# MeteoSwiss/topo-descriptors

Hardware: AMD Instinct MI355X
Metric: Mpixels/s (and % HBM roofline) per descriptor, 1/2/4/8 MI355X (higher is better)
Workload: dtype f32

## Files before the change

### topo_descriptors_amd/csrc/disc_ring_wide_impl.hpp

```cpp
#pragma once

namespace topo {

namespace {

constexpr int NCW = 6;

template <int SIZE>
struct WGeo {
    static constexpr DiscTable<SIZE> T = make_disc_table<SIZE>();
    static_assert(T.centre == 0 && T.off_min == -T.off_max, "odd disc sizes only");
    static constexpr int M = T.off_max;
    static constexpr int DL = (M + NCW - 1) / NCW;
    static constexpr int NVL = 64 - 2 * DL;
    static constexpr int TILE_W = NCW * NVL;
    static constexpr int X0 = NCW * DL;
    static constexpr int W = 64 * NCW;
    static constexpr int NR = T.num_runs;
    static_assert(NVL >= 16, "disc too wide for one wavefront");
    struct Sched {
        int first_step[SIZE];
        int order[SIZE];
        int centre_run;
    };
    static constexpr Sched make() {
        Sched t{};
        for (int r = 0; r < SIZE; ++r) t.first_step[r] = -1;
        for (int r = 0; r < SIZE; ++r) t.order[r] = 0;
        t.centre_run = -1;
        for (int D = 0; D <= DL; ++D)
            for (int s = 0; s < NCW; ++s)
                for (int q = 0; q < NCW; ++q) {
                    const int dr = NCW * D + s - q, dl = -NCW * D + s - q;
                    if (dr >= 0 && dr <= M) {
                        const int r = T.run_of[dr - T.off_min];
                        if (D > t.first_step[r]) t.first_step[r] = D;
                    }
                    if (dl < 0 && dl >= -M) {
                        const int r = T.run_of[dl - T.off_min];
                        if (D > t.first_step[r]) t.first_step[r] = D;
                    }
                }
        int n = 0;
        for (int D = DL; D >= 0; --D)
            for (int d = M; d >= 0; --d) {
                const int r = T.run_of[d - T.off_min];
                bool seen = false;
                for (int i = 0; i < n; ++i) seen = seen || t.order[i] == r;
                if (!seen && t.first_step[r] == D) t.order[n++] = r;
            }
        for (int r = 0; r < NR; ++r)
            if (T.run_lo[r] == 0 && T.run_hi[r] == 0) t.centre_run = r;
        return t;
    }
    static constexpr Sched S = make();
    static_assert(S.centre_run >= 0, "the disc's outermost column is the pixel's own row");
};

template <int SIZE>
struct WideCfg {
    using G = WGeo<SIZE>;
    static constexpr int SW = 3;
    static constexpr int CW = 8;
    static constexpr int NW = SW + CW;
    static constexpr int RPW = 2;
    static constexpr int B = CW * RPW;
    static constexpr int TH = 64;
    static constexpr int PPT = TH / B;
    static constexpr int R = SIZE + 2 * B;
    static constexpr int HALO = SIZE - 1;
    static constexpr int PAD = 1 + (B - (1 + HALO + B) % B) % B;
    static constexpr int PRO = PAD + HALO + B;
    static constexpr int NB_PRO = PRO / B;
    static constexpr size_t LDS = (size_t)R * G::W * sizeof(uint32_t) + 2 * SW * sizeof(int) + 16;
    static_assert(SW * 128 == G::W, "two staged columns per staging lane");
    static_assert(TH % B == 0 && PRO % B == 0, "whole batches");
    static_assert(LDS <= 160 * 1024, "ring does not fit LDS");
    static_assert(NB_PRO <= 15, "batch history: two fields of a flag word");
};

constexpr bool tpi_wide_ring_fits(int size) {
    return size >= 5 && size % 2 == 1 && (size_t)(size + 32) * 384 * 4 + 64 <= 160 * 1024 && 64 - 2 * ((size / 2 + 5) / 6) >= 16;
}

__device__ __forceinline__ int wide_dword_of_column(int c) {
    const int l = c / NCW, s = c - NCW * l;
    return s < 4 ? 4 * l + s : 256 + 2 * l + (s - 4);
}

#ifndef WIDE_LEAD
#define WIDE_LEAD 2
#endif
#ifndef WIDE_PRIO
#define WIDE_PRIO 1
#endif

typedef uint32_t u32x2w __attribute__((ext_vector_type(2)));

template <int SIZE, int R, int LEAD>
__device__ __forceinline__ void wide_disc_sum(const uint32_t* ring, int s0, int lane, uint32_t (&acc)[NCW], uint32_t (&ctr)[NCW], bool first) {
    using G = WGeo<SIZE>;
    constexpr int NR = G::NR;
    constexpr int DL = G::DL;
    constexpr int M = G::M;
    constexpr uint32_t PB = (uint32_t)G::W * 4;
    constexpr uint32_t RB = (uint32_t)R * PB;
    u32x4 top4[NR], bot4[NR];
    u32x2w top2[NR], bot2[NR];
    uint32_t cv[NR][NCW];
    uint32_t aR[NCW], aL[NCW];
    const char* col4 = reinterpret_cast<const char*>(ring + lane * 4);
    const char* col2 = reinterpret_cast<const char*>(ring + 256 + lane * 2);
    const uint32_t b0 = (uint32_t)s0 * PB;
    auto fetch = [&](int i) {
        const int r = G::S.order[i];
        const uint32_t dt = (uint32_t)(G::T.run_hi[r] + 1 + M) * PB, db = (uint32_t)(G::T.run_lo[r] + M) * PB;
        const uint32_t ot = min(b0 + dt, b0 + dt - RB), ob = min(b0 + db, b0 + db - RB);
        top4[r] = *reinterpret_cast<const u32x4*>(col4 + ot);
        top2[r] = *reinterpret_cast<const u32x2w*>(col2 + ot);
        bot4[r] = *reinterpret_cast<const u32x4*>(col4 + ob);
        bot2[r] = *reinterpret_cast<const u32x2w*>(col2 + ob);
    };
#pragma unroll
    for (int i = 0; i < LEAD && i < NR; ++i) fetch(i);
#if WIDE_PRIO
    if (first) CHAIN_SETPRIO(3);
    else CHAIN_SETPRIO(1);
#endif
#pragma unroll
    for (int D = DL; D >= 0; --D) {
#if WIDE_PRIO
        if (D == DL / 2) {
            if (first) CHAIN_SETPRIO(2);
            else CHAIN_SETPRIO(0);
        }
#endif
#pragma unroll
        for (int j = 0; j < NR; ++j) {
            if (G::S.first_step[G::S.order[j]] == D) {
                const int r = G::S.order[j];
                if (j + LEAD < NR) fetch(j + LEAD);
                RING_SB();
#pragma unroll
                for (int s = 0; s < 4; ++s) cv[r][s] = top4[r][s] - bot4[r][s];
#pragma unroll
                for (int s = 0; s < 2; ++s) cv[r][4 + s] = top2[r][s] - bot2[r][s];
                RING_SB();
            }
        }
#pragma unroll
        for (int t = 0; t < NCW; ++t) {
            uint32_t pr = 0, pl = 0;
            bool anyr = false, anyl = false;
#pragma unroll
            for (int s = 0; s < NCW; ++s) {
                const int dr = NCW * D + s - t;
                const int dl = -NCW * D + s - t;
                if (dr >= 0 && dr <= M) {
                    const uint32_t c = cv[G::T.run_of[dr - G::T.off_min]][s];
                    pr = anyr ? pr + c : c;
                    anyr = true;
                }
                if (dl < 0 && dl >= -M) {
                    const uint32_t c = cv[G::T.run_of[dl - G::T.off_min]][s];
                    pl = anyl ? pl + c : c;
                    anyl = true;
                }
            }
            if (D == DL) {
                aR[t] = pr;
                aL[t] = pl;
            } else {
                if (anyr) {
                    asm("" : "+v"(pr));
                    aR[t] = hop(aR[t]) + pr;
                } else {
                    aR[t] = hop(aR[t]);
                }
                if (anyl) {
                    asm("" : "+v"(pl));
                    aL[t] = hop_up(aL[t]) + pl;
                } else {
                    aL[t] = hop_up(aL[t]);
                }
            }
        }
        RING_SB();
    }
#pragma unroll
    for (int t = 0; t < NCW; ++t) {
        acc[t] = aR[t] + aL[t];
        ctr[t] = cv[G::S.centre_run][t];
    }
}


template <int SIZE>
__global__ __launch_bounds__(WideCfg<SIZE>::NW * 64) void tpi_ring_wide_kernel(WaveArgs p, int tiles_x, int tiles_y, PartRun deal) {
    using G = WGeo<SIZE>;
    using C = WideCfg<SIZE>;
    constexpr int B = C::B, R = C::R, PPT = C::PPT, SW = C::SW, NB_PRO = C::NB_PRO, DL = G::DL;
    constexpr unsigned kWindow = (1u << NB_PRO) - 1u;
    constexpr int kBad = 1, kFracOnly = 1 << 15;
    constexpr unsigned kHistMask = kWindow | kWindow * kFracOnly;
    extern __shared__ __attribute__((aligned(16))) uint32_t lds_u[];
    uint32_t* Q = lds_u;
    int* wflags = reinterpret_cast<int*>(Q + R * G::W);

    const int nb = (int)gridDim.x;
    const int vb = (nb & 7) ? (int)blockIdx.x : (int)(blockIdx.x & 7) * (nb >> 3) + (int)(blockIdx.x >> 3);
    const int lane = threadIdx.x & 63;
    const int wave = __builtin_amdgcn_readfirstlane((int)(threadIdx.x >> 6));
    const int ntiles = tiles_x * tiles_y;
    const int first = deal.first(vb);
    const int last = min(first + deal.count(vb), ntiles);
    const double inv_nm1 = 1.0 / ((double)G::T.taps - 1.0);
    const int rmin = max(0, p.in_row0), rmax = min(p.gny, p.in_row0 + p.in_rows);
    const bool stager = wave < SW;
    const int scol = 128 * wave + 2 * lane;
    const int sdw0 = wide_dword_of_column(scol), sdw1 = wide_dword_of_column(scol + 1);
    int seen_tiles = 0, seen_frac = 0;

#pragma unroll 1
    for (int pos = first; pos < last;) {
        const int tile0 = pos;
        const int ty0 = tile0 % tiles_y;
        const int run_tiles = min(last - tile0, tiles_y - ty0);
        const int strip = tile0 / tiles_y;
        const int nphase = run_tiles * PPT;
        const int ox0 = strip * G::TILE_W;
        const int oyS = (p.out_row0 / C::TH + ty0) * C::TH;
        const int gx0 = ox0 - G::X0;
        const int gy0 = oyS - G::M - C::PAD;
        const int gcol = gx0 + scol;
        const bool col_ok = stager && gcol >= 0 && gcol < p.nx;
        const float* src = p.in + (col_ok ? gcol : 0);
        auto load_batch = [&](int n0, float2 (&v)[B]) {
#pragma unroll
            for (int r = 0; r < B; ++r) {
                int gy = gy0 + n0 + r;
                gy = min(max(gy, rmin), rmax - 1);
                v[r] = *reinterpret_cast<const float2*>(src + (size_t)(gy - p.in_row0) * p.nx);
            }
        };
        uint32_t run0 = 0, run1 = 0;
        int wslot = 0;
        const uint32_t kLimBits = __float_as_uint(kAbsLim + 1.0f);
        auto stage_batch = [&](int n0, const float2 (&v)[B]) {
            uint32_t amax = 0;
            bool frac = false;
#pragma unroll
            for (int r = 0; r < B; ++r) {
                const int gy = gy0 + n0 + r;
                const bool ok = col_ok && gy >= rmin && gy < rmax;
                const float x0 = ok ? v[r].x : 0.0f, x1 = ok ? v[r].y : 0.0f;
                const int i0 = (int)x0, i1 = (int)x1;
                const uint32_t a0 = __float_as_uint(x0) & 0x7fffffffu, a1 = __float_as_uint(x1) & 0x7fffffffu;
                frac |= x0 != (float)i0 || x1 != (float)i1;
                amax = max(amax, max(a0, a1));
                run0 += (uint32_t)i0;
                run1 += (uint32_t)i1;
                int sl = wslot + r;
                sl = sl >= R ? sl - R : sl;
                Q[sl * G::W + sdw0] = run0;
                Q[sl * G::W + sdw1] = run1;
            }
            const bool wild = __builtin_amdgcn_ballot_w64(amax >= kLimBits) != 0;
            const bool any_frac = __builtin_amdgcn_ballot_w64(frac) != 0;
            const bool bad = wild || any_frac;
            const bool fr = !wild && any_frac;
            return (bad ? kBad : 0) | (fr ? kFracOnly : 0);
        };
        auto advance_wslot = [&]() {
            wslot += B;
            wslot = wslot >= R ? wslot - R : wslot;
        };
        unsigned hist = 0;
        auto fold = [&](int parity) {
            int all = 0;
#pragma unroll
            for (int w = 0; w < SW; ++w) all |= wflags[parity * SW + w];
            all = __builtin_amdgcn_readfirstlane(all);
            hist = ((hist << 1) | (unsigned)all) & kHistMask;
        };

        float2 va[B];
        __syncthreads();
        if (stager) {
            int bits = 0;
#pragma unroll 1
            for (int k = 0; k < NB_PRO; ++k) {
                load_batch(k * B, va);
                bits |= stage_batch(k * B, va) << (NB_PRO - 1 - k);
                advance_wslot();
            }
            if (lane == 0) wflags[wave] = bits;
            load_batch(C::PRO, va);
        } else {
            for (int k = 0; k < NB_PRO; ++k) advance_wslot();
        }
        __syncthreads();
        {
            int all = 0;
#pragma unroll
            for (int w = 0; w < SW; ++w) all |= wflags[w];
            hist = (unsigned)__builtin_amdgcn_readfirstlane(all) & kHistMask;
        }

        const int ocol = gx0 + lane * NCW;
        const bool lane_ok = lane >= DL && lane < DL + G::NVL && ocol < p.nx;
        bool tile_frac = false;
#pragma unroll 1
        for (int ph = 0; ph < nphase; ++ph) {
            const bool compute = (hist & kWindow) == 0;
            const int oyA = oyS + ph * B;
            tile_frac = tile_frac || (hist & (kWindow * kFracOnly)) != 0;
            if (!compute) {
                const int r0 = max(oyA, p.out_row0), r1 = min(oyA + B, p.out_row0 + p.out_rows) - 1;
                if (r0 <= r1 && threadIdx.x == 0) {
                    const int base = p.out_row0 / p.map_th;
                    const int mx0 = ox0 / p.map_tw, mx1 = (min(ox0 + G::TILE_W, p.nx) - 1) / p.map_tw;
                    for (int mx = mx0; mx <= mx1; ++mx)
                        for (int my = r0 / p.map_th; my <= r1 / p.map_th; ++my) p.defer[mx * p.map_tiles_y + (my - base)] = kNeedsFraction;
                }
            }
            if (ph % PPT == PPT - 1) {
                ++seen_tiles;
                seen_frac += tile_frac ? 1 : 0;
                tile_frac = false;
            }
            if (stager) {
                const int seen = stage_batch(C::PRO + ph * B, va);
                if (lane == 0) wflags[((ph + 1) & 1) * SW + wave] = seen;
                load_batch(C::PRO + (ph + 1) * B, va);
            } else if (compute) {
#pragma unroll 1
                for (int k = 0; k < C::RPW; ++k) {
                    const int j = (wave - SW) * C::RPW + k;
                    const int oy = oyA + j;
                    if (oy < p.out_row0 || oy >= p.out_row0 + p.out_rows) continue;
                    const int s0 = (C::PAD - 1 + ph * B + j) % R;
                    uint32_t acc[NCW], ctr[NCW];
                    wide_disc_sum<SIZE, R, WIDE_LEAD>(Q, s0, lane, acc, ctr, k == 0);
                    if (lane_ok) {
                        float* o = p.tpi + (size_t)(oy - p.out_row0) * p.nx + ocol;
                        float out_t[NCW];
#pragma unroll
                        for (int t = 0; t < NCW; ++t) {
                            const int xi = (int)ctr[t];
                            out_t[t] = (float)((double)xi - (double)((int)acc[t] - xi) * inv_nm1);
                        }
#pragma unroll
                        for (int P = 0; P < NCW / 2; ++P)
                            if (ocol + 2 * P < p.nx) *reinterpret_cast<float2*>(o + 2 * P) = make_float2(out_t[2 * P], out_t[2 * P + 1]);
                    }
                }
            }
            advance_wslot();
            __syncthreads();
            fold((ph + 1) & 1);
        }
        pos += run_tiles;
    }
    if (p.report != nullptr && vb == nb / 2 && threadIdx.x == 0) {
        __hip_atomic_store(p.report + 1, (uint32_t)seen_frac, __ATOMIC_RELAXED, __HIP_MEMORY_SCOPE_SYSTEM);
        __hip_atomic_store(p.report, (uint32_t)seen_tiles, __ATOMIC_RELAXED, __HIP_MEMORY_SCOPE_SYSTEM);
    }
}

template <int SIZE>
int launch_ring_wide(const Block& b, float* tpi_out, int map_th, int map_tw) {
    using G = WGeo<SIZE>;
    using C = WideCfg<SIZE>;
    Context& c = ctx();
    TOPO_REQUIRE(c.seams.n == 0, "the wide ring takes single-block calls only");
    WaveArgs a{b.in, tpi_out, nullptr, b.in_rows, b.in_row0, b.gny, b.nx, b.out_row0, b.out_rows,
               nullptr, nullptr, nullptr, 0, 0, 0};
    static int blocks_per_cu = 0;
    if (blocks_per_cu == 0) {
        TOPO_HIP(hipFuncSetAttribute((const void*)tpi_ring_wide_kernel<SIZE>, hipFuncAttributeMaxDynamicSharedMemorySize, (int)C::LDS));
        int nblk = 0;
        TOPO_HIP(hipOccupancyMaxActiveBlocksPerMultiprocessor(&nblk, (const void*)tpi_ring_wide_kernel<SIZE>, C::NW * 64, C::LDS));
        blocks_per_cu = nblk < 1 ? 1 : nblk;
    }
    a.report = dem_memo_report(b);
    WaveParts ps;
    int tiles_x = 0;
    long ntiles = 0;
    TOPO_TRY(make_parts(b, a, C::TH, G::TILE_W, true, false, &ps, &tiles_x, &ntiles, map_th, map_tw));
    TOPO_REQUIRE(ps.n == 1 && ps.a[0].map_th == map_th && ps.a[0].map_tw == map_tw, "wide ring: tile map of another geometry");
    const size_t map_bytes = (size_t)((b.nx + map_tw - 1) / map_tw) * ps.a[0].map_tiles_y;
    TOPO_HIP(hipMemsetAsync(ps.a[0].defer, kTileDone, map_bytes, c.compute));
    const long grid = march_grid(c, blocks_per_cu, ntiles);
    deal_parts(&ps, tiles_x, grid, blocks_per_cu);
    hipLaunchKernelGGL(tpi_ring_wide_kernel<SIZE>, dim3((unsigned)grid), dim3(C::NW * 64), C::LDS, c.compute, ps.a[0], tiles_x, ps.tiles_y[0], ps.run[0]);
    TOPO_HIP(hipGetLastError());
    return TOPO_AMD_OK;
}

}

}
```

Before: 287,100.

## Share LDS base addresses across disc reads with a mirrored ring guard band

Stores each pixel's six columns contiguously in the LDS ring instead of in a split 4+2 dword layout. Adds GR guard rows that mirror the first ring rows, so nearby row reads can use one shared base register plus a constant offset with no per-read wrap. It also fuses the final left/right chain hop into a single step, turns the first-row flag into a template parameter and fully unrolls the two-row loop. The cost is extra LDS for the guard rows and duplicate stores for those rows, which narrows which disc sizes fit. The LDS reads change from 16+8-byte vector loads to three 8-byte volatile loads.

```diff
diff --git a/topo_descriptors_amd/csrc/disc_ring_wide_impl.hpp b/topo_descriptors_amd/csrc/disc_ring_wide_impl.hpp
--- a/topo_descriptors_amd/csrc/disc_ring_wide_impl.hpp
+++ b/topo_descriptors_amd/csrc/disc_ring_wide_impl.hpp
@@ -68,11 +68,12 @@
     static constexpr int TH = 64;
     static constexpr int PPT = TH / B;
     static constexpr int R = SIZE + 2 * B;
+    static constexpr int GR = 6;
     static constexpr int HALO = SIZE - 1;
     static constexpr int PAD = 1 + (B - (1 + HALO + B) % B) % B;
     static constexpr int PRO = PAD + HALO + B;
     static constexpr int NB_PRO = PRO / B;
-    static constexpr size_t LDS = (size_t)R * G::W * sizeof(uint32_t) + 2 * SW * sizeof(int) + 16;
+    static constexpr size_t LDS = (size_t)(R + GR) * G::W * sizeof(uint32_t) + 2 * SW * sizeof(int) + 16;
     static_assert(SW * 128 == G::W, "two staged columns per staging lane");
     static_assert(TH % B == 0 && PRO % B == 0, "whole batches");
     static_assert(LDS <= 160 * 1024, "ring does not fit LDS");
@@ -80,13 +81,56 @@
 };
 
 constexpr bool tpi_wide_ring_fits(int size) {
-    return size >= 5 && size % 2 == 1 && (size_t)(size + 32) * 384 * 4 + 64 <= 160 * 1024 && 64 - 2 * ((size / 2 + 5) / 6) >= 16;
-}
-
-__device__ __forceinline__ int wide_dword_of_column(int c) {
-    const int l = c / NCW, s = c - NCW * l;
-    return s < 4 ? 4 * l + s : 256 + 2 * l + (s - 4);
-}
+    return size >= 5 && size % 2 == 1 && (size_t)(size + 32 + 6) * 384 * 4 + 64 <= 160 * 1024 && 64 - 2 * ((size / 2 + 5) / 6) >= 16;
+}
+
+template <int SIZE, int GR>
+struct WBase {
+    using G = WGeo<SIZE>;
+    static constexpr int NR = G::NR;
+    struct Tab {
+        int nb;
+        int kb[2 * SIZE];
+        int first[2 * SIZE];
+        int top_b[SIZE], bot_b[SIZE];
+        int top_k[SIZE], bot_k[SIZE];
+    };
+    static constexpr Tab make() {
+        Tab t{};
+        bool need[2 * SIZE + 2] = {};
+        for (int i = 0; i < NR; ++i) {
+            const int r = G::S.order[i];
+            t.top_k[i] = G::T.run_hi[r] + 1 + G::M;
+            t.bot_k[i] = G::T.run_lo[r] + G::M;
+            need[t.top_k[i]] = need[t.bot_k[i]] = true;
+        }
+        t.nb = 0;
+        for (int k = 0; k <= 2 * G::M + 1; ++k)
+            if (need[k] && (t.nb == 0 || k > t.kb[t.nb - 1] + GR)) t.kb[t.nb++] = k;
+        for (int b = 0; b < t.nb; ++b) t.first[b] = NR;
+        auto base_of = [&](int k) {
+            int b = 0;
+            while (b + 1 < t.nb && t.kb[b + 1] <= k) ++b;
+            return b;
+        };
+        for (int i = 0; i < NR; ++i) {
+            t.top_b[i] = base_of(t.top_k[i]);
+            t.bot_b[i] = base_of(t.bot_k[i]);
+            if (i < t.first[t.top_b[i]]) t.first[t.top_b[i]] = i;
+            if (i < t.first[t.bot_b[i]]) t.first[t.bot_b[i]] = i;
+        }
+        return t;
+    }
+    static constexpr Tab T = make();
+    static constexpr bool check() {
+        for (int i = 0; i < NR; ++i)
+            if (T.top_k[i] - T.kb[T.top_b[i]] > GR || T.top_k[i] < T.kb[T.top_b[i]] || T.bot_k[i] - T.kb[T.bot_b[i]] > GR ||
+                T.bot_k[i] < T.kb[T.bot_b[i]])
+                return false;
+        return true;
+    }
+    static_assert(check(), "every read within GR rows of its base");
+};
 
 #ifndef WIDE_LEAD
 #define WIDE_LEAD 2
@@ -96,42 +140,52 @@
 #endif
 
 typedef uint32_t u32x2w __attribute__((ext_vector_type(2)));
-
-template <int SIZE, int R, int LEAD>
-__device__ __forceinline__ void wide_disc_sum(const uint32_t* ring, int s0, int lane, uint32_t (&acc)[NCW], uint32_t (&ctr)[NCW], bool first) {
+typedef __attribute__((address_space(3))) const char lds_char;
+typedef __attribute__((address_space(3))) const volatile u32x2w lds_u32x2w;
+
+template <int SIZE, int R, int GR, int LEAD, bool FIRST>
+__device__ __forceinline__ void wide_disc_sum(const uint32_t* ring, int s0, int lane, uint32_t (&acc)[NCW], uint32_t (&ctr)[NCW]) {
     using G = WGeo<SIZE>;
+    using BT = WBase<SIZE, GR>;
     constexpr int NR = G::NR;
     constexpr int DL = G::DL;
     constexpr int M = G::M;
     constexpr uint32_t PB = (uint32_t)G::W * 4;
     constexpr uint32_t RB = (uint32_t)R * PB;
-    u32x4 top4[NR], bot4[NR];
-    u32x2w top2[NR], bot2[NR];
+    u32x2w top[NR][3], bot[NR][3];
     uint32_t cv[NR][NCW];
     uint32_t aR[NCW], aL[NCW];
-    const char* col4 = reinterpret_cast<const char*>(ring + lane * 4);
-    const char* col2 = reinterpret_cast<const char*>(ring + 256 + lane * 2);
-    const uint32_t b0 = (uint32_t)s0 * PB;
+    uint32_t vb[BT::T.nb];
+    lds_char* q = (lds_char*)ring;
+    const uint32_t b0 = (uint32_t)s0 * PB, lb = (uint32_t)lane * (NCW * 4);
     auto fetch = [&](int i) {
         const int r = G::S.order[i];
-        const uint32_t dt = (uint32_t)(G::T.run_hi[r] + 1 + M) * PB, db = (uint32_t)(G::T.run_lo[r] + M) * PB;
-        const uint32_t ot = min(b0 + dt, b0 + dt - RB), ob = min(b0 + db, b0 + db - RB);
-        top4[r] = *reinterpret_cast<const u32x4*>(col4 + ot);
-        top2[r] = *reinterpret_cast<const u32x2w*>(col2 + ot);
-        bot4[r] = *reinterpret_cast<const u32x4*>(col4 + ob);
-        bot2[r] = *reinterpret_cast<const u32x2w*>(col2 + ob);
+#pragma unroll
+        for (int b = 0; b < BT::T.nb; ++b)
+            if (BT::T.first[b] == i) {
+                const uint32_t d = b0 + (uint32_t)BT::T.kb[b] * PB;
+                vb[b] = lb + min(d, d - RB);
+                asm("" : "+v"(vb[b]));
+            }
+        lds_char* pt = q + vb[BT::T.top_b[i]] + (uint32_t)(BT::T.top_k[i] - BT::T.kb[BT::T.top_b[i]]) * PB;
+        lds_char* pb = q + vb[BT::T.bot_b[i]] + (uint32_t)(BT::T.bot_k[i] - BT::T.kb[BT::T.bot_b[i]]) * PB;
+#pragma unroll
+        for (int h = 0; h < 3; ++h) top[r][h] = *(lds_u32x2w*)(pt + 8 * h);
+#pragma unroll
+        for (int h = 0; h < 3; ++h) bot[r][h] = *(lds_u32x2w*)(pb + 8 * h);
     };
 #pragma unroll
     for (int i = 0; i < LEAD && i < NR; ++i) fetch(i);
 #if WIDE_PRIO
-    if (first) CHAIN_SETPRIO(3);
+    if (FIRST) CHAIN_SETPRIO(3);
     else CHAIN_SETPRIO(1);
 #endif
+    static_assert(DL >= 1, "the last step (D = 0) closes both chains");
 #pragma unroll
     for (int D = DL; D >= 0; --D) {
 #if WIDE_PRIO
         if (D == DL / 2) {
-            if (first) CHAIN_SETPRIO(2);
+            if (FIRST) CHAIN_SETPRIO(2);
             else CHAIN_SETPRIO(0);
         }
 #endif
@@ -142,9 +196,7 @@
                 if (j + LEAD < NR) fetch(j + LEAD);
                 RING_SB();
 #pragma unroll
-                for (int s = 0; s < 4; ++s) cv[r][s] = top4[r][s] - bot4[r][s];
-#pragma unroll
-                for (int s = 0; s < 2; ++s) cv[r][4 + s] = top2[r][s] - bot2[r][s];
+                for (int s = 0; s < NCW; ++s) cv[r][s] = top[r][s / 2][s % 2] - bot[r][s / 2][s % 2];
                 RING_SB();
             }
         }
@@ -170,6 +222,13 @@
             if (D == DL) {
                 aR[t] = pr;
                 aL[t] = pl;
+            } else if (D == 0) {
+                uint32_t own = anyr && anyl ? pr + pl : anyr ? pr : pl;
+                asm("" : "+v"(own));
+                own = hop_up(aL[t]) + own;
+                asm("" : "+v"(own));
+                aR[t] = hop(aR[t]) + own;
+                asm("" : "+v"(aR[t]));
             } else {
                 if (anyr) {
                     asm("" : "+v"(pr));
@@ -189,7 +248,7 @@
     }
 #pragma unroll
     for (int t = 0; t < NCW; ++t) {
-        acc[t] = aR[t] + aL[t];
+        acc[t] = aR[t];
         ctr[t] = cv[G::S.centre_run][t];
     }
 }
@@ -205,7 +264,7 @@
     constexpr unsigned kHistMask = kWindow | kWindow * kFracOnly;
     extern __shared__ __attribute__((aligned(16))) uint32_t lds_u[];
     uint32_t* Q = lds_u;
-    int* wflags = reinterpret_cast<int*>(Q + R * G::W);
+    int* wflags = reinterpret_cast<int*>(Q + (R + C::GR) * G::W);
 
     const int nb = (int)gridDim.x;
     const int vb = (nb & 7) ? (int)blockIdx.x : (int)(blockIdx.x & 7) * (nb >> 3) + (int)(blockIdx.x >> 3);
@@ -218,7 +277,6 @@
     const int rmin = max(0, p.in_row0), rmax = min(p.gny, p.in_row0 + p.in_rows);
     const bool stager = wave < SW;
     const int scol = 128 * wave + 2 * lane;
-    const int sdw0 = wide_dword_of_column(scol), sdw1 = wide_dword_of_column(scol + 1);
     int seen_tiles = 0, seen_frac = 0;
 
 #pragma unroll 1
@@ -262,8 +320,9 @@
                 run1 += (uint32_t)i1;
                 int sl = wslot + r;
                 sl = sl >= R ? sl - R : sl;
-                Q[sl * G::W + sdw0] = run0;
-                Q[sl * G::W + sdw1] = run1;
+                const u32x2w v2 = {run0, run1};
+                *reinterpret_cast<u32x2w*>(Q + sl * G::W + scol) = v2;
+                if (sl < C::GR) *reinterpret_cast<u32x2w*>(Q + (sl + R) * G::W + scol) = v2;
             }
             const bool wild = __builtin_amdgcn_ballot_w64(amax >= kLimBits) != 0;
             const bool any_frac = __builtin_amdgcn_ballot_w64(frac) != 0;
@@ -334,14 +393,16 @@
                 if (lane == 0) wflags[((ph + 1) & 1) * SW + wave] = seen;
                 load_batch(C::PRO + (ph + 1) * B, va);
             } else if (compute) {
-#pragma unroll 1
+                static_assert(C::RPW == 2, "two rows per chain wave: the first and the second priority pair");
+#pragma unroll
                 for (int k = 0; k < C::RPW; ++k) {
                     const int j = (wave - SW) * C::RPW + k;
                     const int oy = oyA + j;
                     if (oy < p.out_row0 || oy >= p.out_row0 + p.out_rows) continue;
                     const int s0 = (C::PAD - 1 + ph * B + j) % R;
                     uint32_t acc[NCW], ctr[NCW];
-                    wide_disc_sum<SIZE, R, WIDE_LEAD>(Q, s0, lane, acc, ctr, k == 0);
+                    if (k == 0) wide_disc_sum<SIZE, R, C::GR, WIDE_LEAD, true>(Q, s0, lane, acc, ctr);
+                    else wide_disc_sum<SIZE, R, C::GR, WIDE_LEAD, false>(Q, s0, lane, acc, ctr);
                     if (lane_ok) {
                         float* o = p.tpi + (size_t)(oy - p.out_row0) * p.nx + ocol;
                         float out_t[NCW];
```

Result: faster. 303,900 (median of 6 runs) (+5.8%).
